# dominikh/jello

Hardware: AMD Instinct MI355X
Metric: Mpixels/sec fine-raster + paths/sec, 100k-path 4096^2 scene (higher is better)
Workload: dtype f32

## Files before the change

include/jello_hip.h:

```cpp
#ifndef JELLO_HIP_H
#define JELLO_HIP_H

#include <stddef.h>
#include <stdint.h>

#ifdef __cplusplus
extern "C" {
#endif

typedef struct jh_ctx jh_ctx;

typedef enum jh_status {
    JH_OK = 0,
    JH_ERR_INVALID = -1,
    JH_ERR_DEVICE = -2,
    JH_ERR_NO_DEVICE = -3,
    JH_ERR_UNSUPPORTED = -4,
    JH_ERR_OOM = -5
} jh_status;

typedef enum jh_stage {
    JH_PATHTAG_REDUCE = 0,
    JH_PATHTAG_REDUCE2 = 1,
    JH_PATHTAG_SCAN1 = 2,
// ... 99 lines not shown
typedef struct jh_yuv_desc {
    int32_t layout, matrix, range, transfer;
    void* plane[3];
    uint64_t pitch[3];
} jh_yuv_desc;
int jh_blit_yuv(jh_ctx* ctx, uint64_t src_image_id, uint32_t width, uint32_t height, const jh_yuv_desc* desc);

uint64_t jh_pack_bound(uint32_t width, uint32_t height, uint32_t texel_bytes);
int jh_pack_tiles(jh_ctx* ctx, const void* src, uint64_t src_pitch, const void* ref , uint64_t ref_pitch, uint32_t width,
                  uint32_t height, uint32_t texel_bytes, void* dst, uint64_t dst_capacity);
int jh_unpack_tiles(jh_ctx* ctx, const void* pack, uint64_t pack_bytes, void* dst, uint64_t dst_pitch, uint32_t width, uint32_t height,
                    uint32_t texel_bytes);
int jh_debug_unpack_rejects(jh_ctx* ctx, uint32_t* count, int reset);

typedef struct jh_dash_el { int32_t kind, pad; double pts[6]; } jh_dash_el;
typedef struct jh_dash_path { uint32_t first_el, n_els, first_dash, n_dash; double offset; } jh_dash_path;
typedef struct jh_dash_out_el { uint32_t kind; float p[6]; } jh_dash_out_el;
int jh_dash(jh_ctx* ctx, const jh_dash_el* els, uint64_t n_els, const jh_dash_path* paths, uint32_t n_paths, const double* dashes,
            uint64_t n_dashes, void* out_els, uint64_t out_capacity, uint32_t* out_index);

int jh_profile_enable(jh_ctx* ctx, int on);
int jh_profile_collect(jh_ctx* ctx, jh_profile_record* out, int max);
int jh_profile_group_begin(jh_ctx* ctx, const char* label);
int jh_profile_group_end(jh_ctx* ctx);
int jh_profile_collect_tree(jh_ctx* ctx, jh_profile_node* out, int max);

int jh_selftest_math(jh_ctx* ctx, int op, const float* a, const float* b, float* out, uint32_t n);
int jh_selftest_atomics(jh_ctx* ctx, int form, uint32_t seed, uint32_t n_waves);
uint64_t jh_debug_scratch_bytes(jh_ctx* ctx, int slot);
int jh_scratch_trim(jh_ctx* ctx);
int jh_debug_flatten_regions(jh_ctx* ctx, uint32_t flags);
uint64_t jh_debug_graph_self_cleans(jh_ctx* ctx);
int jh_debug_poison_scratch(jh_ctx* ctx, int byte);

int jh_device_info(jh_ctx* ctx, char* name, int name_len, int* compute_units, uint64_t* total_mem);
uint64_t jh_pool_bytes(jh_ctx* ctx);

#ifdef __cplusplus
}
#endif
#endif
```

jello_amd/_lib.py:

```python
import ctypes
import os
import subprocess

_HERE = os.path.dirname(os.path.abspath(__file__))
_ROOT = os.path.dirname(_HERE)


class HostLibraryMissing(RuntimeError):
    pass


def lib_paths():
    return {
        "hip": os.environ.get("JELLO_HIP_LIB") or os.path.join(_HERE, "libjello_hip.so"),
        "host": os.environ.get("JELLO_HOST_LIB") or os.path.join(_HERE, "libjello_host.so"),
    }


def build(verbose=False):
    for sub in ("csrc", "host"):
        cmd = ["make", "-C", os.path.join(_HERE, sub), "-j8"]
        r = subprocess.run(cmd, stdout=subprocess.PIPE, stderr=subprocess.STDOUT, text=True)
        if verbose or r.returncode != 0:
            print(r.stdout)
# ... 179 lines not shown
    hip.jh_image_create.argtypes = [vp, ctypes.c_uint64, ctypes.c_uint32, ctypes.c_uint32, ci]
    hip.jh_image_upload.argtypes = [vp, ctypes.c_uint64, ctypes.c_uint32, ctypes.c_uint32, ci, vp, ctypes.c_uint64]
    hip.jh_image_free.argtypes = [vp, ctypes.c_uint64]
    hip.jh_blit.argtypes = [vp, ctypes.c_uint64, vp, ctypes.c_uint64, ctypes.c_uint32, ctypes.c_uint32, ci]
    hip.jh_blit_yuv.argtypes = [vp, ctypes.c_uint64, ctypes.c_uint32, ctypes.c_uint32, ctypes.POINTER(CYuvDesc)]
    hip.jh_pack_bound.restype = u64
    hip.jh_pack_bound.argtypes = [u32, u32, u32]
    hip.jh_pack_tiles.argtypes = [vp, vp, u64, vp, u64, u32, u32, u32, vp, u64]
    hip.jh_unpack_tiles.argtypes = [vp, vp, u64, vp, u64, u32, u32, u32]
    hip.jh_dash.argtypes = [vp, ctypes.POINTER(PathEl), u64, ctypes.POINTER(CDashPath), u32, dp, u64, vp, u64, vp]
    hip.jh_debug_unpack_rejects.argtypes = [vp, ctypes.POINTER(u32), ci]
    hip.jh_image_write.argtypes = [vp, ctypes.c_uint64, ctypes.c_uint32, ctypes.c_uint32, ctypes.c_uint32, ctypes.c_uint32, vp, ctypes.c_uint64]
    hip.jh_buffer_import.argtypes = [vp, ctypes.c_uint64, vp, ctypes.c_uint64]
    hip.jh_graph_begin.argtypes = [vp]
    hip.jh_graph_end.argtypes = [vp, ctypes.POINTER(vp)]
    hip.jh_graph_launch.argtypes = [vp, vp]
    hip.jh_graph_node_counts.argtypes = [vp, vp, ctypes.POINTER(ctypes.c_uint32), ctypes.POINTER(ctypes.c_uint32)]
    hip.jh_graph_destroy.argtypes = [vp, vp]
    hip.jh_free.argtypes = [vp, ctypes.c_uint64]
    hip.jh_clear.argtypes = [vp, ctypes.c_uint64, ctypes.c_uint64, ctypes.c_int64]
    hip.jh_pool_bytes.restype = ctypes.c_uint64
    hip.jh_pool_bytes.argtypes = [vp]
    hip.jh_device_info.argtypes = [vp, ctypes.c_char_p, ci, ctypes.POINTER(ci), ctypes.POINTER(ctypes.c_uint64)]
    hip.jh_debug_poison_scratch.argtypes = [vp, ci]
    hip.jh_debug_scratch_bytes.restype = ctypes.c_uint64
    hip.jh_debug_scratch_bytes.argtypes = [vp, ci]
    if hasattr(hip, "jh_debug_flatten_regions"):
        hip.jh_debug_flatten_regions.restype = ci
        hip.jh_debug_flatten_regions.argtypes = [vp, ctypes.c_uint32]
    if hasattr(hip, "jh_scratch_trim"):
        hip.jh_scratch_trim.restype = ci
        hip.jh_scratch_trim.argtypes = [vp]
    hip.jh_set_clip_depth_hint.argtypes = [vp, ctypes.c_uint32]
    if hasattr(hip, "jh_debug_clip_hint_overflows"):
        hip.jh_debug_clip_hint_overflows.argtypes = [vp, ctypes.POINTER(ctypes.c_uint32), ctypes.c_int]
    hip.jh_debug_graph_self_cleans.restype = ctypes.c_uint64
    hip.jh_debug_graph_self_cleans.argtypes = [vp]
```

jello_amd/csrc/jello_hip.cpp:

```cpp
#include "../../include/jello_hip.h"

#include <hip/hip_runtime.h>

#include <algorithm>
#include <chrono>
#include <cstdlib>
#include <cstdio>
#include <cstring>
#include <map>
#include <string>
#include <unordered_map>
#include <vector>

#include "kcommon.h"
#include "../../include/jello_dash_host.h"

#ifndef JH_SCR_SKEW
#define JH_SCR_SKEW 1280u
#endif
enum { JH_CLEAN_FL_CTR = 1u, JH_CLEAN_BD_CTR = 2u, JH_CLEAN_SCAN = 8u, JH_CLEAN_PC_TOT = 16u };
static const struct { int slot; uint32_t flag; } kSelfCleaned[] = {
    {JH_SCR_FL_CTR, JH_CLEAN_FL_CTR}, {JH_SCR_BD_CTR, JH_CLEAN_BD_CTR}, {JH_SCR_SCAN_TMP, JH_CLEAN_SCAN}, {JH_SCR_PC_TOT, JH_CLEAN_PC_TOT}};
static uint32_t clean_flag_of(int slot) {
    for (const auto& k : kSelfCleaned)
// ... 1240 lines not shown
    if (b) HIP_TRY(ctx, hipMemcpyAsync(db, b, bytes, hipMemcpyHostToDevice, ctx->stream));
    int rc = jh_selftest_math_launch(ctx->stream, op, da, db, dout, n);
    if (rc == 0) {
        HIP_TRY(ctx, hipMemcpyAsync(out, dout, bytes, hipMemcpyDeviceToHost, ctx->stream));
        HIP_TRY(ctx, hipStreamSynchronize(ctx->stream));
    }
    (void)hipFree(da); (void)hipFree(dout);
    if (db) (void)hipFree(db);
    return rc == 0 ? JH_OK : fail(ctx, JH_ERR_DEVICE, "selftest launch failed");
}

int jh_selftest_atomics_launch(hipStream_t stream, int form, uint32_t seed, uint32_t n_waves);

int jh_selftest_atomics(jh_ctx* ctx, int form, uint32_t seed, uint32_t n_waves) {
    if (!ctx) return JH_ERR_INVALID;
    JH_FLUSH(ctx);
    HIP_TRY(ctx, hipSetDevice(ctx->device));
    const int rc = jh_selftest_atomics_launch(ctx->stream, form, seed, n_waves);
    if (rc == -1) return fail(ctx, JH_ERR_INVALID, "selftest_atomics: form 0..2, 1..4096 waves");
    if (rc < 0) return fail(ctx, JH_ERR_DEVICE, "selftest_atomics: runtime error");
    return rc;
}

int jh_debug_poison_scratch(jh_ctx* ctx, int byte) {
    if (!ctx) return JH_ERR_INVALID;
    JH_FLUSH(ctx);
    HIP_TRY(ctx, hipSetDevice(ctx->device));
    for (int i = 0; i < JH_SCR_COUNT; i++)
        if (ctx->scratch.ptr[i] && ctx->scratch.cap[i]) HIP_TRY(ctx, hipMemsetAsync(ctx->scratch.ptr[i], byte, ctx->scratch.cap[i], ctx->stream));
    ctx->scratch.clean_flags = 0u;
    return JH_OK;
}

int jh_set_clip_depth_hint(jh_ctx* ctx, uint32_t max_depth) {
    if (!ctx) return JH_ERR_INVALID;
    ctx->clip_depth_hint = max_depth;
    return JH_OK;
}
int jh_debug_flatten_regions(jh_ctx* ctx, uint32_t flags) {
    if (!ctx) return JH_ERR_INVALID;
    ctx->debug_flatten = flags;
    ctx->generation++;
    return JH_OK;
}
int jh_debug_clip_hint_overflows(jh_ctx* ctx, uint32_t* count, int reset) {
    if (!ctx || !ctx->hint_overflow) return JH_ERR_INVALID;
    JH_FLUSH(ctx);
    HIP_TRY(ctx, hipStreamSynchronize(ctx->stream));
    if (count) {
        HIP_TRY(ctx, hipMemcpyAsync(count, ctx->hint_overflow, 4, hipMemcpyDeviceToHost, ctx->stream));
        HIP_TRY(ctx, hipStreamSynchronize(ctx->stream));
    }
    if (reset) {
        HIP_TRY(ctx, hipMemsetAsync(ctx->hint_overflow, 0, 4, ctx->stream));
        HIP_TRY(ctx, hipStreamSynchronize(ctx->stream));
    }
    return JH_OK;
}
#ifdef FINE_TIMING
extern "C" int jh_debug_fine_timing(jh_ctx* ctx, unsigned long long* out6, int reset) {
    if (!ctx || !ctx->hint_overflow) return JH_ERR_INVALID;
    HIP_TRY(ctx, hipStreamSynchronize(ctx->stream));
    if (out6) { HIP_TRY(ctx, hipMemcpyAsync(out6, ctx->hint_overflow + 8, 48, hipMemcpyDeviceToHost, ctx->stream)); HIP_TRY(ctx, hipStreamSynchronize(ctx->stream)); }
    if (reset) { HIP_TRY(ctx, hipMemsetAsync(ctx->hint_overflow + 8, 0, 48, ctx->stream)); HIP_TRY(ctx, hipStreamSynchronize(ctx->stream)); }
    return JH_OK;
}
// ... 44 lines not shown
```

jello_amd/csrc/kernels_fine.hip:

```cpp
#include <cstring>

#include "kcommon.h"
#include <algorithm>
#include "srgb_lut.h"

using namespace jk;
using namespace jd;

namespace {

struct V4 {
    float x, y, z, w;
};
struct V3 {
    float x, y, z;
};
JD V4 v4(float x, float y, float z, float w) { V4 r; r.x = x; r.y = y; r.z = z; r.w = w; return r; }
JD V3 v3(float x, float y, float z) { V3 r; r.x = x; r.y = y; r.z = z; return r; }

JD V3 screen(V3 cb, V3 cs) { return v3(cb.x + cs.x - (cb.x * cs.x), cb.y + cs.y - (cb.y * cs.y), cb.z + cs.z - (cb.z * cs.z)); }
JD float color_dodge(float cb, float cs) {
    if (cb == 0.0f) return 0.0f; else if (cs == 1.0f) return 1.0f; else return fmin_(1.0f, cb / (1.0f - cs));
}
JD float color_burn(float cb, float cs) {
    if (cb == 1.0f) return 1.0f; else if (cs == 0.0f) return 0.0f; else return 1.0f - fmin_(1.0f, (1.0f - cb) / cs);
}
JD float hard_light1(float cb, float cs) {
    float scr_cs = 2.0f * cs - 1.0f;
    float a = cb + scr_cs - (cb * scr_cs);
    float b = cb * 2.0f * cs;
    return (cs <= 0.5f) ? b : a;
}
JD V3 hard_light(V3 cb, V3 cs) { return v3(hard_light1(cb.x, cs.x), hard_light1(cb.y, cs.y), hard_light1(cb.z, cs.z)); }
JD float soft_light1(float cb, float cs) {
    float d = (cb <= 0.25f) ? (((16.0f * cb - 12.0f) * cb + 4.0f) * cb) : sqrt_(cb);
    float t = cb + (2.0f * cs - 1.0f) * (d - cb);
// ... 119 lines not shown
typedef float jk_v4f __attribute__((ext_vector_type(4)));
typedef float jk_v2f __attribute__((ext_vector_type(2)));
#if defined(__HIP_DEVICE_COMPILE__)
JD float4 lds_ld_f4(uint32_t a) { const jk_v4f v = *(const JK_LDS jk_v4f*)a; return make_float4(v.x, v.y, v.z, v.w); }
JD void lds_st_u16(uint32_t a, uint16_t v) { *(JK_LDS uint16_t*)a = v; }
JD void lds_st_u8(uint32_t a, uint8_t v) { *(JK_LDS uint8_t*)a = v; }
JD float lds_ld_f32(uint32_t a) { return *(const JK_LDS float*)a; }
#else
JD float4 lds_ld_f4(uint32_t) { return make_float4(0.0f, 0.0f, 0.0f, 0.0f); }
JD void lds_st_u16(uint32_t, uint16_t) {}
JD void lds_st_u8(uint32_t, uint8_t) {}
JD float lds_ld_f32(uint32_t) { return 0.0f; }
#endif

JD V4 over(V4 bg, V4 fg, float area) {
    V4 fg_i = v4(fg.x * area, fg.y * area, fg.z * area, fg.w * area);
    float k = 1.0f - fg_i.w;
    return v4(bg.x * k + fg_i.x, bg.y * k + fg_i.y, bg.z * k + fg_i.z, bg.w * k + fg_i.w);
}

#define FB_SPEC 128u
#ifndef FINE_LEAN_WAVES_PER_EU
#define FINE_LEAN_WAVES_PER_EU 7
#endif
#ifndef FINE_CLIP_WAVES_PER_EU
#define FINE_CLIP_WAVES_PER_EU 4
#endif
#ifndef FINE_CLIP_MS_WAVES_PER_EU
#define FINE_CLIP_MS_WAVES_PER_EU 3
#endif
#ifndef FINE_WAVES
#define FINE_WAVES 1
#endif
#define FB_PLANE 65
#ifndef FINE_SKIP
#define FINE_SKIP 0
#endif
#if FINE_SKIP != 0 && !defined(JH_VARIANT_BUILD)
#error "FINE_SKIP changes results: build it as a variant library (make VARIANT=name EXTRA='-DJH_VARIANT_BUILD -DFINE_SKIP=n')"
#endif
#define RK_NONEG 1u
#define RK_RANGE 2u
#define RK_LUM 4u
#define FINE_TRIP_WORDS 13u
template <bool LEAN> struct FillLdsT;
template <> struct FillLdsT<false> {
    alignas(16) float4 pre[64];
    alignas(16) float4 ent[4][63];
    float pre_ye[64];
    float edge_y[64];
    int8_t edge_s[64];
    uint64_t rowmask[16];
    uint32_t lanest[64];
    union {
        uint8_t pairflag[64];
        uint8_t specmark[64];
    };
};

template <> struct FillLdsT<true> {
    alignas(16) float4 pre[64];
    alignas(16) float4 ent[4][FB_PLANE];
    float pre_ye[64];
    float2 edge[64];
    uint64_t rowmask[16];
    uint32_t lanest[1];
    uint8_t first[4];
    union {
        uint8_t pairflag[64];
        uint8_t specmark[FB_SPEC];
    };
};
typedef FillLdsT<false> FillLds;
JD void load_segraw_clamped(const float* __restrict__ segments, uint32_t segments_n, uint32_t so, float& p0x, float& p0y, float& p1x,
                            float& p1y, float& ye) {
    const float2* sp = (const float2*)(segments + (size_t)umin_(so, umax_(segments_n, 1u) - 1u) * 6);
    float2 a = sp[0], b = sp[1], c = sp[2];
    p0x = a.x; p0y = a.y; p1x = b.x; p1y = b.y; ye = c.x;
}

#ifdef MS_CAP_OVERRIDE
#define MS_CAP(SAMPLES) MS_CAP_OVERRIDE
#else
#define MS_CAP(SAMPLES) ((SAMPLES) == 8 ? 192u : 256u)
#endif
#define MS_F_DOWN 1u
#define MS_F_BUMP_NZ 2u
#define MS_F_BUMP_EO 4u
#define MS_F_CARRY 8u
#define MS_F_LIVE 16u
#define MS_S_DOWN 1u
#define MS_S_RIGHT 2u
#define MS_S_TOP_ON_EDGE 4u
#define MS_S_BOT_OFF_EDGE 8u
#define MS_S_BY_RULE 16u
struct MsSeg {
    float a, b;
    int32_t x0i;
    float top_y;
    float lut_row;
    uint32_t bits;
    uint32_t first;
};
template <int SAMPLES> struct MsLds {
    union {
// ... 420 lines not shown
    const uint32_t lane = threadIdx.x & 63u;
    const uint32_t ly = lane >> 2, lx = lane & 3u;
    const uint32_t tile_ix = tile_y * (fc.valid ? fc.width_in_tiles : cfg->width_in_tiles) + tile_x;
    const uint32_t scratch_tile = blockIdx.y * tiles_x + tile_x;
    const float xyx = (float)((tile_x * 4u + lx) * 4u);
    const float xyy = (float)(tile_y * 16u + ly);
    V4 rgba[4];
#pragma unroll
    for (int k = 0; k < 4; k++)
        rgba[k] = fc.valid ? v4(fc.base_color[0], fc.base_color[1], fc.base_color[2], fc.base_color[3])
                           : v4(cfg->base_color[0], cfg->base_color[1], cfg->base_color[2], cfg->base_color[3]);
    uint32_t clip_depth = 0u;
    uint32_t pushed_depth = 0u;
    float area[4] = {0.0f, 0.0f, 0.0f, 0.0f};
    uint32_t pc = uni(tile_ix * JL_PTCL_INITIAL_ALLOC);
    MsState msb;
    msb.base = 0u; msb.hi = 0u; msb.next = 0xffffffffu; msb.total = 0u; msb.direct = false; msb.first = 0u; msb.edge = 0u; msb.clean = 2u;
    auto I = [&](uint32_t i) -> uint32_t { return i < info_n ? info[i] : 0u; };
    const uint32_t blend_offset = pc < ptcl_n ? ptcl[pc] : 0u;
    pc += 1u;
    auto load_grad = [&](int32_t x, uint32_t y) -> V4 {
        if (x < 0 || x >= JL_GRADIENT_WIDTH || y >= grad_h) return v4(0, 0, 0, 0);
        const uint16_t* t = gradients + ((size_t)y * JL_GRADIENT_WIDTH + (size_t)x) * 4;
        uint2 raw = *(const uint2*)t;
        return v4(f16_to_f32((uint16_t)(raw.x & 0xffffu)), f16_to_f32((uint16_t)(raw.x >> 16)), f16_to_f32((uint16_t)(raw.y & 0xffffu)),
                  f16_to_f32((uint16_t)(raw.y >> 16)));
    };
    auto pix_i = [&](int k) -> float { return (float)k; };
    auto pix_spill = [&](int k) -> uint32_t { return ly * JL_TILE_WIDTH + lx * 4u + (uint32_t)k; };
    uint32_t cur_base = 0u, nxt_base = 0xffffffffu;
    uint32_t batch_hi = 0u;
    uint32_t n_pairs = 0u;
    uint64_t edge_mask = 0ull;
    uint32_t next_seg = 0xffffffffu;
    const float lyf = (float)ly;
    uint32_t ent_lds = 0u;
    uint64_t s4_rowmask = 0ull;
    uint32_t s4_first = 0u, s4_row_addr = 0u, s4_done = 0u;
    if constexpr (AA == 0) ent_lds = lds_addr(&F.ent[lx][0]);

    auto build_batch = [&](uint32_t so) {
      if constexpr (AA == 0) {
        wave_sync();
        float c_p0x, c_p0y, c_p1x, c_p1y, c_ye;
        if (nxt_base == so) {
            __builtin_amdgcn_s_waitcnt(0x0F70);
            wave_sync();
            const float4 t = lds_ld_f4(lds_addr(&F.pre[lane]));
            c_p0x = t.x; c_p0y = t.y; c_p1x = t.z; c_p1y = t.w; c_ye = lds_ld_f32(lds_addr(&F.pre_ye[lane]));
        } else {
            load_segraw_clamped(segments, segments_n, so + lane, c_p0x, c_p0y, c_p1x, c_p1y, c_ye);
        }
        {
            const bool ok = so + lane < segments_n;
            c_p0x = ok ? c_p0x : 0.0f; c_p0y = ok ? c_p0y : 0.0f; c_p1x = ok ? c_p1x : 0.0f; c_p1y = ok ? c_p1y : 0.0f;
            c_ye = ok ? c_ye : 0.0f;
        }
        cur_base = so;
        const float dlx = c_p1x - c_p0x, dly = c_p1y - c_p0y;
        if constexpr (CLIPS) { F.edge_y[lane] = c_ye; F.edge_s[lane] = (int8_t)(dlx > 0.0f ? 1 : (dlx < 0.0f ? -1 : 0)); }
        else F.edge[lane] = make_float2(c_ye, sign_(dlx));
        const bool sane = abs_(c_p0x) <= 64.0f && abs_(c_p0y) <= 64.0f && abs_(c_p1x) <= 64.0f && abs_(c_p1y) <= 64.0f;
        int32_t ra = 0, rb = 16;
        if (sane) {
            ra = iclamp_((int32_t)floor_(fmin_(c_p0y, c_p1y) - 1.0e-3f), 0, 16);
            rb = iclamp_((int32_t)ceil_(fmax_(c_p0y, c_p1y) + 1.0e-3f), 0, 16);
        }
        const uint32_t my_cnt = (uint32_t)imax_(rb - ra, 0);
        const uint32_t incl = wave_incl_scan_u32(my_cnt);
        const uint64_t fit = __builtin_amdgcn_ballot_w64(incl <= 63u) & 0x7fffffffffffffffull;
        const uint32_t e_rel = (uint32_t)__builtin_popcountll(fit);
        n_pairs = (uint32_t)__builtin_amdgcn_readlane((int)incl, (int)(e_rel - 1u));
        const uint32_t first = incl - my_cnt;
        if constexpr (!CLIPS) s4_first = lane < e_rel ? first : n_pairs;
        edge_mask = __builtin_amdgcn_ballot_w64(c_ye < 16.0f) & fit;
        const uint32_t meta = first | ((uint32_t)ra << 8) | (sane ? (1u << 16) : 0u);
        nxt_base = so + e_rel;
        {
            const float* gp = segments + (size_t)umin_(nxt_base + lane, umax_(segments_n, 1u) - 1u) * 6;
            __builtin_amdgcn_global_load_lds((const __attribute__((address_space(1))) void*)gp, (JK_LDS void*)&F.pre[0], 16, 0, 0);
            __builtin_amdgcn_global_load_lds((const __attribute__((address_space(1))) void*)(gp + 4), (JK_LDS void*)&F.pre_ye[0], 4, 0, 0);
        }
        F.pairflag[lane] = 0u;
        if (lane < 16u) F.rowmask[lane] = 0ull;
        batch_hi = so + e_rel;
#if FINE_SKIP == 6
        {
            next_seg = so;
            const bool is_pair = lane < n_pairs;
            const float y = c_p0y - (float)(ra & 15);
            const float y0 = clamp_(y, 0.0f, 1.0f);
            const float y1 = clamp_(y + dly, 0.0f, 1.0f);
            const float s2_dy = y0 - y1;
            const float vec_y_recip = 1.0f / dly;
            const float s2_tx0 = ((y0 - y) * vec_y_recip) * dlx, s2_tx1 = ((y1 - y) * vec_y_recip) * dlx;
            const float gx0 = c_p0x + s2_tx0, gx1 = c_p0x + s2_tx1;
            const float xmin0 = fmin_(gx0, gx1), xmax0 = fmax_(gx0, gx1);
            const bool guard = sane && abs_(xmin0) <= 40.0f && abs_(xmax0) <= 40.0f;
            const int32_t c1 = guard ? iclamp_((int32_t)ceil_(xmax0 + 1.0e-3f), 0, 16) : 16;
            const int32_t n0 = guard ? iclamp_((int32_t)floor_(xmin0 - 1.0e-3f), 0, 16) : 0;
            const uint32_t ncross = (is_pair && s2_dy != 0.0f) ? (uint32_t)imax_(c1 - n0, 0) : 0u;
            const uint32_t nspec = wave_reduce_u32(ncross);
            float sink = 0.0f;
            for (uint32_t k0 = 0u; k0 < nspec; k0 += 64u) {
                const uint32_t X = ((uint32_t)n0 + k0) & 15u;
                const float i_f = (float)(X & 3u);
                const float startx = c_p0x - (float)(4u * (X >> 2));
                const float x0 = startx + s2_tx0, x1 = startx + s2_tx1;
                const float xmn0 = fmin_(x0, x1), xmx0 = fmax_(x0, x1);
                float xmin = fmin_(xmn0 - i_f, 1.0f) - 1.0e-6f;
                float xmax = xmx0 - i_f;
                float b = fmin_(xmax, 1.0f);
                float c = fmax_(b, 0.0f);
                float d = fmax_(xmin, 0.0f);
                float a = (b + 0.5f * (d * d - c * c) - xmin) / (xmax - xmin);
                sink = a * s2_dy;
                asm volatile("" : "+v"(sink));
            }
            asm volatile("" ::"v"(sink));
            return;
        }
#endif
        wave_sync();
        if (lane < e_rel && my_cnt != 0u) F.pairflag[first & 63u] = lane + 1u;
        wave_sync();
        const uint32_t owner = wave_incl_max_u32(F.pairflag[lane]);
        const uint32_t pseg = (owner - 1u) & 63u;
        const uint32_t pmeta = __shfl(meta, (int)pseg, 64);
        const float p0x = __shfl(c_p0x, (int)pseg, 64), p0y = __shfl(c_p0y, (int)pseg, 64);
        const float sdx = __shfl(dlx, (int)pseg, 64), sdy = __shfl(dly, (int)pseg, 64);
        const bool is_pair = FINE_SKIP == 3 ? false : lane < n_pairs;
        const uint32_t row = is_pair ? ((((pmeta >> 8) & 31u) + (lane - (pmeta & 0xffu))) & 15u) : 0u;
        const float y = p0y - (float)row;
        const float y0 = clamp_(y, 0.0f, 1.0f);
        const float y1 = clamp_(y + sdy, 0.0f, 1.0f);
        const float s2_dy = y0 - y1;
        const float vec_y_recip = 1.0f / sdy;
        const float t0 = (y0 - y) * vec_y_recip;
        const float t1 = (y1 - y) * vec_y_recip;
        const float s2_tx0 = t0 * sdx, s2_tx1 = t1 * sdx;
        const float gx0 = p0x + s2_tx0, gx1 = p0x + s2_tx1;
        const float xmin0 = fmin_(gx0, gx1), xmax0 = fmax_(gx0, gx1);
        const bool guard = (pmeta & (1u << 16)) != 0u && abs_(xmin0) <= 40.0f && abs_(xmax0) <= 40.0f;
        const int32_t c1 = guard ? iclamp_((int32_t)ceil_(xmax0 + 1.0e-3f), 0, 16) : 16;
        const int32_t n0 = guard ? iclamp_((int32_t)floor_(xmin0 - 1.0e-3f), 0, 16) : 0;
        const uint32_t ncross = (is_pair && s2_dy != 0.0f) ? (uint32_t)imax_(c1 - n0, 0) : 0u;
        if (is_pair) atomicOr((unsigned long long*)&F.rowmask[row], 1ull << lane);
        wave_sync();
        const uint64_t rm_pair = F.rowmask[row];
        const uint32_t rank = __builtin_amdgcn_mbcnt_hi((uint32_t)(rm_pair >> 32), __builtin_amdgcn_mbcnt_lo((uint32_t)rm_pair, 0u));
        const uint32_t c16 = (uint32_t)__builtin_popcountll(F.rowmask[lane & 15u]);
        uint32_t inc16 = c16;
        inc16 += (uint32_t)__builtin_amdgcn_update_dpp(0, (int)inc16, JK_DPP_ROW_SHR(1), 0xf, 0xf, false);
        inc16 += (uint32_t)__builtin_amdgcn_update_dpp(0, (int)inc16, JK_DPP_ROW_SHR(2), 0xf, 0xf, false);
        inc16 += (uint32_t)__builtin_amdgcn_update_dpp(0, (int)inc16, JK_DPP_ROW_SHR(4), 0xf, 0xf, false);
        inc16 += (uint32_t)__builtin_amdgcn_update_dpp(0, (int)inc16, JK_DPP_ROW_SHR(8), 0xf, 0xf, false);
        const uint32_t excl16 = inc16 - c16;
        const uint32_t pos = (__shfl(excl16, (int)row, 64) + rank) & 63u;
        if constexpr (CLIPS) {
            F.lanest[lane] = (ent_lds + __shfl(excl16, (int)ly, 64) * 16u) | ((lane < e_rel ? first : n_pairs) << 24);
        } else {
            s4_row_addr = ent_lds + __shfl(excl16, (int)ly, 64) * 16u;
            s4_done = 0u;
            s4_rowmask = F.rowmask[ly];
        }
        next_seg = so;
        if (is_pair) {
            const float c1f = (float)c1;
            float cv[16];
#pragma unroll
            for (int q = 0; q < 16; q++) cv[q] = clamp_((float)(q + 1) - c1f, 0.0f, 1.0f) * s2_dy;
#pragma unroll
            for (int q = 0; q < 4; q++) F.ent[q][pos] = make_float4(cv[4 * q], cv[4 * q + 1], cv[4 * q + 2], cv[4 * q + 3]);
        }
        if (ncross != 0u) {
            const uint32_t X = (uint32_t)n0 & 15u;
            const float i_f = (float)(X & 3u);
            const float startx = p0x - (float)(4u * (X >> 2));
            const float x0 = startx + s2_tx0, x1 = startx + s2_tx1;
            const float xmn0 = fmin_(x0, x1), xmx0 = fmax_(x0, x1);
            float xmin = fmin_(xmn0 - i_f, 1.0f) - 1.0e-6f;
            float xmax = xmx0 - i_f;
            float b = fmin_(xmax, 1.0f);
            float c = fmax_(b, 0.0f);
            float d = fmax_(xmin, 0.0f);
            float a = (b + 0.5f * (d * d - c * c) - xmin) / (xmax - xmin);
            ((float*)&F.ent[X >> 2][pos])[X & 3u] = a * s2_dy;
        }
        const uint32_t nrest = ncross != 0u ? ncross - 1u : 0u;
        const int32_t n0r = n0 + 1;
        const uint32_t sincl = wave_incl_scan_u32(nrest);
        const uint32_t spos = sincl - nrest;
        const uint32_t nspec = (FINE_SKIP == 1 || FINE_SKIP == 3) ? 0u : (uint32_t)__builtin_amdgcn_readlane((int)sincl, 63);
        const uint32_t packed = ((uint32_t)n0r & 15u) | (pos << 4) | (spos << 10);
        constexpr uint32_t SPEC = (uint32_t)sizeof(F.specmark);
        for (uint32_t pass = 0u; pass < nspec; pass += SPEC) {
            wave_sync();
            if constexpr (SPEC == 128u) ((uint16_t*)F.specmark)[lane] = 0u; else F.specmark[lane] = 0u;
            wave_sync();
            if (nrest != 0u && spos - pass < SPEC) F.specmark[spos - pass] = (uint8_t)(lane + 1u);
            wave_sync();
            const uint64_t before = __builtin_amdgcn_ballot_w64(nrest != 0u && spos < pass);
            uint32_t carry = before != 0ull ? 64u - (uint32_t)__builtin_clzll(before) : 0u;
            const uint32_t n_here = umin_(nspec - pass, SPEC);
            for (uint32_t k0 = 0u; k0 < n_here; k0 += 64u) {
                const uint32_t own = umax_(wave_incl_max_u32(F.specmark[k0 + lane]), carry);
                carry = (uint32_t)__builtin_amdgcn_readlane((int)own, 63);
                const uint32_t j = (own - 1u) & 63u;
                const float dy = __shfl(s2_dy, (int)j, 64), tx0 = __shfl(s2_tx0, (int)j, 64), tx1 = __shfl(s2_tx1, (int)j, 64);
                const float q0x = __shfl(p0x, (int)j, 64);
                const uint32_t pk = __shfl(packed, (int)j, 64);
                if (k0 + lane < n_here) {
                    const uint32_t X = ((pk & 15u) + (pass + k0 + lane - (pk >> 10))) & 15u;
                    const uint32_t epos = (pk >> 4) & 63u;
                    const uint32_t g = X >> 2;
                    const float i_f = (float)(X & 3u);
                    const float startx = q0x - (float)(4u * g);
                    const float x0 = startx + tx0, x1 = startx + tx1;
                    const float xmn0 = fmin_(x0, x1), xmx0 = fmax_(x0, x1);
                    float xmin = fmin_(xmn0 - i_f, 1.0f) - 1.0e-6f;
                    float xmax = xmx0 - i_f;
                    float b = fmin_(xmax, 1.0f);
                    float c = fmax_(b, 0.0f);
                    float d = fmax_(xmin, 0.0f);
                    float a = (b + 0.5f * (d * d - c * c) - xmin) / (xmax - xmin);
                    ((float*)&F.ent[X >> 2][epos])[X & 3u] = a * dy;
                }
            }
        }
        wave_sync();
      } else {
        (void)so;
      }
    };

    auto load_win = [&](uint32_t b) -> uint32_t {
        const uint32_t i = b + lane;
        return (i < ptcl_n && i >= b) ? ptcl[i] : 0u;
    };
    uint32_t wbase = pc;
    uint32_t wcur = load_win(wbase), wnext = load_win(wbase + 64u);
    if (ptcl_head == ~0u) return;
    auto materialize = [&]() {
        if constexpr (CLIPS) {
            while (pushed_depth < clip_depth) {
                if (pushed_depth < FINE_LDS_LEVELS) {
// ... 133 lines not shown
                    asm volatile(
                        "s_mov_b64 %[sv], exec\n"
                        "1:\n"
                        "v_cmpx_lt_u32_e32 vcc, %[cur], %[hi]\n"
                        "s_cbranch_execz 3f\n"
                        "ds_read_b128 v[64:67], %[cur]\n"
                        "v_add_u32_e32 %[t], 16, %[cur]\n"
                        "v_cmp_lt_u32_e32 vcc, %[t], %[hi]\n"
                        "s_mov_b64 %[s1], exec\n"
                        "s_and_b64 exec, exec, vcc\n"
                        "ds_read_b128 v[68:71], %[cur] offset:16\n"
                        "s_mov_b64 exec, %[s1]\n"
                        "v_add_u32_e32 %[cur], 32, %[cur]\n"
                        "s_waitcnt lgkmcnt(1)\n"
                        "v_pk_add_f32 %[a01], %[a01], v[64:65]\n"
                        "v_pk_add_f32 %[a23], %[a23], v[66:67]\n"
                        "s_and_b64 exec, exec, vcc\n"
                        "s_waitcnt lgkmcnt(0)\n"
                        "v_pk_add_f32 %[a01], %[a01], v[68:69]\n"
                        "v_pk_add_f32 %[a23], %[a23], v[70:71]\n"
                        "s_mov_b64 exec, %[s1]\n"
                        "s_branch 1b\n"
                        "3:\n"
                        "s_mov_b64 exec, %[sv]\n"
                        : [cur] "+v"(cur), [a01] "+v"(a01), [a23] "+v"(a23), [sv] "=&s"(sv), [s1] "=&s"(s1), [t] "=&v"(t)
                        : [hi] "v"(hi)
                        : "vcc", "memory", "v64", "v65", "v66", "v67", "v68", "v69", "v70", "v71");
                    area[0] = a01.x; area[1] = a01.y; area[2] = a23.x; area[3] = a23.y;
                }
                cur = hi;
                if (em == 0ull) break;
                {
                    float2 ed;
                    if constexpr (CLIPS) ed = make_float2(F.edge_y[e_sl], (float)F.edge_s[e_sl]); else ed = F.edge[e_sl];
                    const float y_edge = ed.y * clamp_(lyf - ed.x + 1.0f, 0.0f, 1.0f);
                    area[0] += y_edge; area[1] += y_edge; area[2] += y_edge; area[3] += y_edge;
                }
                em &= em - 1ull;
            }
            if constexpr (CLIPS) lds_st_u8(lds_addr(&F.lanest[lane]) + 2u, (uint8_t)done); else s4_done = done;
#ifdef FINE_TIMING
            tm_walk += __builtin_readcyclecounter() - tb1;
#endif
            next_seg = sa + take;
            sa += take;
            remaining -= take;
        }
        if (even_odd) {
#pragma unroll
            for (int k = 0; k < 4; k++) { float a = area[k]; area[k] = abs_(a - 2.0f * round_(0.5f * a)); }
        } else {
#pragma unroll
            for (int k = 0; k < 4; k++) {
#if defined(__HIP_DEVICE_COMPILE__)
                asm("v_min_f32_e64 %0, |%1|, 1.0" : "=v"(area[k]) : "v"(area[k]));
#else
                area[k] = fmin_(abs_(area[k]), 1.0f);
#endif
            }
        }
      } else {
        (void)n_segs; (void)even_odd;
        ms_fill<AA>(F, msb, lane, size_and_rule, seg_data, backdrop, segments, segments_n, mask_lut, mask_lut_n, area);
      }
    };
    auto ensure_window = [&]() {
    if (pc - wbase > 64u - FINE_TRIP_WORDS) {
// ... 408 lines not shown
        fc.width_in_tiles = L.cfg_host->width_in_tiles;
        for (int i = 0; i < 4; i++) fc.base_color[i] = L.cfg_host->base_color[i];
    }
    float4* clip_scratch = nullptr;
    uint32_t scr_levels = 0u;
    if (clips) {
        scr_levels = FINE_SCR_LEVELS;
        if (L.clip_depth_hint != 0u) scr_levels = L.clip_depth_hint > FINE_LDS_LEVELS ? std::min<uint32_t>(L.clip_depth_hint - FINE_LDS_LEVELS, FINE_SCR_LEVELS) : 0u;
        clip_scratch = (float4*)jh_scratch_get(L.scratch, JH_SCR_D, (uint64_t)L.gx * (trow1 - trow0) * scr_levels * 4096u);
        if (!clip_scratch) return JH_L_SCRATCH;
    }
#define JH_FINE_LAUNCH(A, C, P)                                                                                                          \
    hipLaunchKernelGGL((k_fine_area<A, C, P>), dim3((L.gx + FINE_WG_WAVES(C) - 1) / FINE_WG_WAVES(C), trow1 - trow0), dim3(64 * FINE_WG_WAVES(C)), 0, L.stream, cfg, fc, seg_ptr, \
                       segments_n, L.ptr<const uint32_t>(FN_PTCL), ptcl_n, L.ptr<const uint32_t>(FN_INFO), info_n, spill, (uint16_t*)out.ptr,         \
                       out.width, out.height, (const uint16_t*)grad.ptr, grad_h, imgs, L.gx, mask_lut, mask_lut_n, trow0, clip_scratch, scr_levels, L.hint_overflow)
#define JH_FINE_PICK(A)                                  \
    do {                                                 \
        if (clips && paints) JH_FINE_LAUNCH(A, true, true);   \
        else if (clips) JH_FINE_LAUNCH(A, true, false);       \
        else if (paints) JH_FINE_LAUNCH(A, false, true);      \
        else JH_FINE_LAUNCH(A, false, false);                 \
    } while (0)
    if (aa == 8) JH_FINE_PICK(8);
    else if (aa == 16) JH_FINE_PICK(16);
    else JH_FINE_PICK(0);
#undef JH_FINE_PICK
#undef JH_FINE_LAUNCH
    return JH_L_OK;
}

JhResult jh_launch_fine_area(const JhLaunch& L) { return launch_fine(L, 0); }
JhResult jh_launch_fine_msaa8(const JhLaunch& L) { return launch_fine(L, 8); }
JhResult jh_launch_fine_msaa16(const JhLaunch& L) { return launch_fine(L, 16); }
```

Baseline: 21480.

## Shrink lean fine-area LDS window to 32 segments for higher occupancy

New measurement: 21270, median of 2. No clear change (-1.0%).

```diff
diff --git a/include/jello_hip.h b/include/jello_hip.h
--- a/include/jello_hip.h
+++ b/include/jello_hip.h
@@ -155,6 +155,7 @@
 int jh_debug_flatten_regions(jh_ctx* ctx, uint32_t flags);
 uint64_t jh_debug_graph_self_cleans(jh_ctx* ctx);
 int jh_debug_poison_scratch(jh_ctx* ctx, int byte);
+int jh_debug_fine_occupancy(jh_ctx* ctx, int aa, int clips, int paints);
 
 int jh_device_info(jh_ctx* ctx, char* name, int name_len, int* compute_units, uint64_t* total_mem);
 uint64_t jh_pool_bytes(jh_ctx* ctx);
diff --git a/jello_amd/_lib.py b/jello_amd/_lib.py
--- a/jello_amd/_lib.py
+++ b/jello_amd/_lib.py
@@ -235,6 +235,9 @@
         hip.jh_scratch_trim.restype = ci
         hip.jh_scratch_trim.argtypes = [vp]
     hip.jh_set_clip_depth_hint.argtypes = [vp, ctypes.c_uint32]
+    if hasattr(hip, "jh_debug_fine_occupancy"):
+        hip.jh_debug_fine_occupancy.restype = ci
+        hip.jh_debug_fine_occupancy.argtypes = [vp, ci, ci, ci]
     if hasattr(hip, "jh_debug_clip_hint_overflows"):
         hip.jh_debug_clip_hint_overflows.argtypes = [vp, ctypes.POINTER(ctypes.c_uint32), ctypes.c_int]
     hip.jh_debug_graph_self_cleans.restype = ctypes.c_uint64
diff --git a/jello_amd/csrc/jello_hip.cpp b/jello_amd/csrc/jello_hip.cpp
--- a/jello_amd/csrc/jello_hip.cpp
+++ b/jello_amd/csrc/jello_hip.cpp
@@ -1296,6 +1296,16 @@
     return JH_OK;
 }
 
+extern "C" int jh_fine_occupancy_query(int aa, int clips, int paints);
+
+int jh_debug_fine_occupancy(jh_ctx* ctx, int aa, int clips, int paints) {
+    if (!ctx) return JH_ERR_INVALID;
+    HIP_TRY(ctx, hipSetDevice(ctx->device));
+    const int n = jh_fine_occupancy_query(aa, clips, paints);
+    if (n < 0) return fail(ctx, JH_ERR_INVALID, "fine_occupancy: aa 0 / 8 / 16, or the runtime refused the query");
+    return n;
+}
+
 int jh_set_clip_depth_hint(jh_ctx* ctx, uint32_t max_depth) {
     if (!ctx) return JH_ERR_INVALID;
     ctx->clip_depth_hint = max_depth;
diff --git a/jello_amd/csrc/kernels_fine.hip b/jello_amd/csrc/kernels_fine.hip
--- a/jello_amd/csrc/kernels_fine.hip
+++ b/jello_amd/csrc/kernels_fine.hip
@@ -2,6 +2,7 @@
 
 #include "kcommon.h"
 #include <algorithm>
+#include <type_traits>
 #include "srgb_lut.h"
 
 using namespace jk;
@@ -187,7 +188,6 @@
 #ifndef FINE_WAVES
 #define FINE_WAVES 1
 #endif
-#define FB_PLANE 65
 #ifndef FINE_SKIP
 #define FINE_SKIP 0
 #endif
@@ -200,6 +200,7 @@
 #define FINE_TRIP_WORDS 13u
 template <bool LEAN> struct FillLdsT;
 template <> struct FillLdsT<false> {
+    static constexpr uint32_t WIN = 64u;
     alignas(16) float4 pre[64];
     alignas(16) float4 ent[4][63];
     float pre_ye[64];
@@ -213,19 +214,20 @@
     };
 };
 
+#define FINE_LDS_BLOCK 1280u
 template <> struct FillLdsT<true> {
-    alignas(16) float4 pre[64];
-    alignas(16) float4 ent[4][FB_PLANE];
-    float pre_ye[64];
-    float2 edge[64];
+    static constexpr uint32_t WIN = 32u;
+    alignas(16) float4 pre[32];
+    alignas(16) float4 ent[4][63];
+    float pre_ye[32];
+    float edge_y[32];
     uint64_t rowmask[16];
-    uint32_t lanest[1];
-    uint8_t first[4];
     union {
         uint8_t pairflag[64];
         uint8_t specmark[FB_SPEC];
     };
 };
+static_assert(sizeof(FillLdsT<true>) + 16u <= 4u * FINE_LDS_BLOCK, "the lean area kernel must fit four LDS blocks (28 tile-waves per CU)");
 typedef FillLdsT<false> FillLds;
 JD void load_segraw_clamped(const float* __restrict__ segments, uint32_t segments_n, uint32_t so, float& p0x, float& p0y, float& p1x,
                             float& p1y, float& ye) {
@@ -712,6 +714,7 @@
     uint32_t batch_hi = 0u;
     uint32_t n_pairs = 0u;
     uint64_t edge_mask = 0ull;
+    uint32_t edge_pos = 0u, edge_neg = 0u;
     uint32_t next_seg = 0xffffffffu;
     const float lyf = (float)ly;
     uint32_t ent_lds = 0u;
@@ -722,52 +725,62 @@
     auto build_batch = [&](uint32_t so) {
       if constexpr (AA == 0) {
         wave_sync();
+        uint32_t bl = lane;
+        if constexpr (!CLIPS) asm volatile("" : "+v"(bl));
+        constexpr uint32_t W = std::remove_reference_t<decltype(F)>::WIN;
+        constexpr uint64_t WMASK = W == 64u ? 0x7fffffffffffffffull : (1ull << (W & 63u)) - 1ull;
+        const bool in_win = W == 64u || bl < W;
         float c_p0x, c_p0y, c_p1x, c_p1y, c_ye;
         if (nxt_base == so) {
             __builtin_amdgcn_s_waitcnt(0x0F70);
             wave_sync();
-            const float4 t = lds_ld_f4(lds_addr(&F.pre[lane]));
-            c_p0x = t.x; c_p0y = t.y; c_p1x = t.z; c_p1y = t.w; c_ye = lds_ld_f32(lds_addr(&F.pre_ye[lane]));
+            static_assert(sizeof(F.pre) + 64u * 16u <= sizeof(F) && offsetof(std::remove_reference_t<decltype(F)>, pre_ye) + 64u * 4u <= sizeof(F), "all 64 lanes read inside F");
+            const float4 t = lds_ld_f4(lds_addr(&F.pre[0]) + bl * 16u);
+            c_p0x = t.x; c_p0y = t.y; c_p1x = t.z; c_p1y = t.w; c_ye = lds_ld_f32(lds_addr(&F.pre_ye[0]) + bl * 4u);
         } else {
-            load_segraw_clamped(segments, segments_n, so + lane, c_p0x, c_p0y, c_p1x, c_p1y, c_ye);
+            load_segraw_clamped(segments, segments_n, so + bl, c_p0x, c_p0y, c_p1x, c_p1y, c_ye);
         }
         {
-            const bool ok = so + lane < segments_n;
+            const bool ok = in_win && so + bl < segments_n;
             c_p0x = ok ? c_p0x : 0.0f; c_p0y = ok ? c_p0y : 0.0f; c_p1x = ok ? c_p1x : 0.0f; c_p1y = ok ? c_p1y : 0.0f;
             c_ye = ok ? c_ye : 0.0f;
         }
         cur_base = so;
         const float dlx = c_p1x - c_p0x, dly = c_p1y - c_p0y;
-        if constexpr (CLIPS) { F.edge_y[lane] = c_ye; F.edge_s[lane] = (int8_t)(dlx > 0.0f ? 1 : (dlx < 0.0f ? -1 : 0)); }
-        else F.edge[lane] = make_float2(c_ye, sign_(dlx));
+        if constexpr (CLIPS) { F.edge_y[bl] = c_ye; F.edge_s[bl] = (int8_t)(dlx > 0.0f ? 1 : (dlx < 0.0f ? -1 : 0)); }
+        else if (in_win) F.edge_y[bl] = c_ye;
         const bool sane = abs_(c_p0x) <= 64.0f && abs_(c_p0y) <= 64.0f && abs_(c_p1x) <= 64.0f && abs_(c_p1y) <= 64.0f;
         int32_t ra = 0, rb = 16;
         if (sane) {
             ra = iclamp_((int32_t)floor_(fmin_(c_p0y, c_p1y) - 1.0e-3f), 0, 16);
             rb = iclamp_((int32_t)ceil_(fmax_(c_p0y, c_p1y) + 1.0e-3f), 0, 16);
         }
-        const uint32_t my_cnt = (uint32_t)imax_(rb - ra, 0);
+        const uint32_t my_cnt = in_win ? (uint32_t)imax_(rb - ra, 0) : 0u;
         const uint32_t incl = wave_incl_scan_u32(my_cnt);
-        const uint64_t fit = __builtin_amdgcn_ballot_w64(incl <= 63u) & 0x7fffffffffffffffull;
+        const uint64_t fit = __builtin_amdgcn_ballot_w64(incl <= 63u) & WMASK;
         const uint32_t e_rel = (uint32_t)__builtin_popcountll(fit);
         n_pairs = (uint32_t)__builtin_amdgcn_readlane((int)incl, (int)(e_rel - 1u));
         const uint32_t first = incl - my_cnt;
-        if constexpr (!CLIPS) s4_first = lane < e_rel ? first : n_pairs;
+        if constexpr (!CLIPS) s4_first = bl < e_rel ? first : n_pairs;
         edge_mask = __builtin_amdgcn_ballot_w64(c_ye < 16.0f) & fit;
+        if constexpr (!CLIPS) {
+            static_assert(CLIPS || W <= 32u, "edge_pos / edge_neg are 32-bit masks");
+            edge_pos = (uint32_t)(__builtin_amdgcn_ballot_w64(dlx > 0.0f) & edge_mask); edge_neg = (uint32_t)(__builtin_amdgcn_ballot_w64(dlx < 0.0f) & edge_mask);
+        }
         const uint32_t meta = first | ((uint32_t)ra << 8) | (sane ? (1u << 16) : 0u);
         nxt_base = so + e_rel;
-        {
-            const float* gp = segments + (size_t)umin_(nxt_base + lane, umax_(segments_n, 1u) - 1u) * 6;
+        if (in_win) {
+            const float* gp = segments + (size_t)umin_(nxt_base + bl, umax_(segments_n, 1u) - 1u) * 6;
             __builtin_amdgcn_global_load_lds((const __attribute__((address_space(1))) void*)gp, (JK_LDS void*)&F.pre[0], 16, 0, 0);
             __builtin_amdgcn_global_load_lds((const __attribute__((address_space(1))) void*)(gp + 4), (JK_LDS void*)&F.pre_ye[0], 4, 0, 0);
         }
-        F.pairflag[lane] = 0u;
-        if (lane < 16u) F.rowmask[lane] = 0ull;
+        F.pairflag[bl] = 0u;
+        if (bl < 16u) F.rowmask[bl] = 0ull;
         batch_hi = so + e_rel;
 #if FINE_SKIP == 6
         {
             next_seg = so;
-            const bool is_pair = lane < n_pairs;
+            const bool is_pair = bl < n_pairs;
             const float y = c_p0y - (float)(ra & 15);
             const float y0 = clamp_(y, 0.0f, 1.0f);
             const float y1 = clamp_(y + dly, 0.0f, 1.0f);
@@ -802,15 +815,15 @@
         }
 #endif
         wave_sync();
-        if (lane < e_rel && my_cnt != 0u) F.pairflag[first & 63u] = lane + 1u;
+        if (bl < e_rel && my_cnt != 0u) F.pairflag[first & 63u] = bl + 1u;
         wave_sync();
-        const uint32_t owner = wave_incl_max_u32(F.pairflag[lane]);
+        const uint32_t owner = wave_incl_max_u32(F.pairflag[bl]);
         const uint32_t pseg = (owner - 1u) & 63u;
         const uint32_t pmeta = __shfl(meta, (int)pseg, 64);
         const float p0x = __shfl(c_p0x, (int)pseg, 64), p0y = __shfl(c_p0y, (int)pseg, 64);
         const float sdx = __shfl(dlx, (int)pseg, 64), sdy = __shfl(dly, (int)pseg, 64);
-        const bool is_pair = FINE_SKIP == 3 ? false : lane < n_pairs;
-        const uint32_t row = is_pair ? ((((pmeta >> 8) & 31u) + (lane - (pmeta & 0xffu))) & 15u) : 0u;
+        const bool is_pair = FINE_SKIP == 3 ? false : bl < n_pairs;
+        const uint32_t row = is_pair ? ((((pmeta >> 8) & 31u) + (bl - (pmeta & 0xffu))) & 15u) : 0u;
         const float y = p0y - (float)row;
         const float y0 = clamp_(y, 0.0f, 1.0f);
         const float y1 = clamp_(y + sdy, 0.0f, 1.0f);
@@ -825,11 +838,11 @@
         const int32_t c1 = guard ? iclamp_((int32_t)ceil_(xmax0 + 1.0e-3f), 0, 16) : 16;
         const int32_t n0 = guard ? iclamp_((int32_t)floor_(xmin0 - 1.0e-3f), 0, 16) : 0;
         const uint32_t ncross = (is_pair && s2_dy != 0.0f) ? (uint32_t)imax_(c1 - n0, 0) : 0u;
-        if (is_pair) atomicOr((unsigned long long*)&F.rowmask[row], 1ull << lane);
+        if (is_pair) atomicOr((unsigned long long*)&F.rowmask[row], 1ull << bl);
         wave_sync();
         const uint64_t rm_pair = F.rowmask[row];
         const uint32_t rank = __builtin_amdgcn_mbcnt_hi((uint32_t)(rm_pair >> 32), __builtin_amdgcn_mbcnt_lo((uint32_t)rm_pair, 0u));
-        const uint32_t c16 = (uint32_t)__builtin_popcountll(F.rowmask[lane & 15u]);
+        const uint32_t c16 = (uint32_t)__builtin_popcountll(F.rowmask[bl & 15u]);
         uint32_t inc16 = c16;
         inc16 += (uint32_t)__builtin_amdgcn_update_dpp(0, (int)inc16, JK_DPP_ROW_SHR(1), 0xf, 0xf, false);
         inc16 += (uint32_t)__builtin_amdgcn_update_dpp(0, (int)inc16, JK_DPP_ROW_SHR(2), 0xf, 0xf, false);
@@ -838,7 +851,7 @@
         const uint32_t excl16 = inc16 - c16;
         const uint32_t pos = (__shfl(excl16, (int)row, 64) + rank) & 63u;
         if constexpr (CLIPS) {
-            F.lanest[lane] = (ent_lds + __shfl(excl16, (int)ly, 64) * 16u) | ((lane < e_rel ? first : n_pairs) << 24);
+            F.lanest[bl] = (ent_lds + __shfl(excl16, (int)ly, 64) * 16u) | ((bl < e_rel ? first : n_pairs) << 24);
         } else {
             s4_row_addr = ent_lds + __shfl(excl16, (int)ly, 64) * 16u;
             s4_done = 0u;
@@ -876,22 +889,22 @@
         constexpr uint32_t SPEC = (uint32_t)sizeof(F.specmark);
         for (uint32_t pass = 0u; pass < nspec; pass += SPEC) {
             wave_sync();
-            if constexpr (SPEC == 128u) ((uint16_t*)F.specmark)[lane] = 0u; else F.specmark[lane] = 0u;
+            if constexpr (SPEC == 128u) ((uint16_t*)F.specmark)[bl] = 0u; else F.specmark[bl] = 0u;
             wave_sync();
-            if (nrest != 0u && spos - pass < SPEC) F.specmark[spos - pass] = (uint8_t)(lane + 1u);
+            if (nrest != 0u && spos - pass < SPEC) F.specmark[spos - pass] = (uint8_t)(bl + 1u);
             wave_sync();
             const uint64_t before = __builtin_amdgcn_ballot_w64(nrest != 0u && spos < pass);
             uint32_t carry = before != 0ull ? 64u - (uint32_t)__builtin_clzll(before) : 0u;
             const uint32_t n_here = umin_(nspec - pass, SPEC);
             for (uint32_t k0 = 0u; k0 < n_here; k0 += 64u) {
-                const uint32_t own = umax_(wave_incl_max_u32(F.specmark[k0 + lane]), carry);
+                const uint32_t own = umax_(wave_incl_max_u32(F.specmark[k0 + bl]), carry);
                 carry = (uint32_t)__builtin_amdgcn_readlane((int)own, 63);
                 const uint32_t j = (own - 1u) & 63u;
                 const float dy = __shfl(s2_dy, (int)j, 64), tx0 = __shfl(s2_tx0, (int)j, 64), tx1 = __shfl(s2_tx1, (int)j, 64);
                 const float q0x = __shfl(p0x, (int)j, 64);
                 const uint32_t pk = __shfl(packed, (int)j, 64);
-                if (k0 + lane < n_here) {
-                    const uint32_t X = ((pk & 15u) + (pass + k0 + lane - (pk >> 10))) & 15u;
+                if (k0 + bl < n_here) {
+                    const uint32_t X = ((pk & 15u) + (pass + k0 + bl - (pk >> 10))) & 15u;
                     const uint32_t epos = (pk >> 4) & 63u;
                     const uint32_t g = X >> 2;
                     const float i_f = (float)(X & 3u);
@@ -1091,7 +1104,8 @@
                 if (em == 0ull) break;
                 {
                     float2 ed;
-                    if constexpr (CLIPS) ed = make_float2(F.edge_y[e_sl], (float)F.edge_s[e_sl]); else ed = F.edge[e_sl];
+                    if constexpr (CLIPS) ed = make_float2(F.edge_y[e_sl], (float)F.edge_s[e_sl]);
+                    else ed = make_float2(F.edge_y[e_sl], ((edge_pos >> (e_sl & 31u)) & 1u) != 0u ? 1.0f : (((edge_neg >> (e_sl & 31u)) & 1u) != 0u ? -1.0f : 0.0f));
                     const float y_edge = ed.y * clamp_(lyf - ed.x + 1.0f, 0.0f, 1.0f);
                     area[0] += y_edge; area[1] += y_edge; area[2] += y_edge; area[3] += y_edge;
                 }
@@ -1566,3 +1580,22 @@
 JhResult jh_launch_fine_area(const JhLaunch& L) { return launch_fine(L, 0); }
 JhResult jh_launch_fine_msaa8(const JhLaunch& L) { return launch_fine(L, 8); }
 JhResult jh_launch_fine_msaa16(const JhLaunch& L) { return launch_fine(L, 16); }
+
+extern "C" int jh_fine_occupancy_query(int aa, int clips, int paints) {
+    int n = -1;
+    hipError_t e = hipErrorInvalidValue;
+#define JH_FINE_OCC(A, C, P) e = hipOccupancyMaxActiveBlocksPerMultiprocessor(&n, k_fine_area<A, C, P>, 64 * FINE_WG_WAVES(C), 0)
+#define JH_FINE_OCC_PICK(A)                               \
+    do {                                                  \
+        if (clips && paints) JH_FINE_OCC(A, true, true);  \
+        else if (clips) JH_FINE_OCC(A, true, false);      \
+        else if (paints) JH_FINE_OCC(A, false, true);     \
+        else JH_FINE_OCC(A, false, false);                \
+    } while (0)
+    if (aa == 0) JH_FINE_OCC_PICK(0);
+    else if (aa == 8) JH_FINE_OCC_PICK(8);
+    else if (aa == 16) JH_FINE_OCC_PICK(16);
+#undef JH_FINE_OCC_PICK
+#undef JH_FINE_OCC
+    return e == hipSuccess ? n : -1;
+}
```
